# nilspin/VoxelHashing_demo

Measured on AMD Instinct MI355X. Metric: frames/s TSDF-integrated + raycast Mpix/s, 640×480, 1/2/4/8 MI355X, higher is better.
Workload: dtype f32

## Files before the change

voxelhashing_demo_amd/csrc/vh_api.hip:

```cpp
#include <hip/hip_runtime.h>
#include <hip/hip_ext.h>
#include <dlfcn.h>

#include <algorithm>
#include <chrono>
#include <cmath>
#include <cstdio>
#include <cstdlib>
#include <cstring>
#include <string>
#include <type_traits>
#include <utility>
#include <vector>

#include "vh_kernels.hip"

using namespace vh;

static thread_local std::string g_last_error;

static int fail(int code, const char *what, hipError_t e = hipSuccess)
{
    g_last_error = what;
    if (e != hipSuccess) {
// ... 143 lines not shown
    std::vector<std::pair<hipEvent_t, hipEvent_t>> eventPool;
    uint64_t profiledFrames = 0;
    vh_kernel_times times{};
    int integrateGrid = 2048;
    void *raycastStamps = nullptr;
    int raycastBeam = 3;
    int raycastMode = VH_RAYCAST_DDA;
    int packetFormat = VH_PACKET_F32;
    int fusedFrame = 1;
    int commitBlocks = 128;
    int fusedParity = 0;
    bool compactArmed = false;
    int flattenVariant = 4;
    int walkReverse = 1;
    uint32_t walkBackward = 0;
    uint32_t candAllocated = 0;
    uint32_t allocEpoch = 0;
    uint32_t epochTotal = 0;
    DevBuf<float> fusedPlane;
    int pipeline = 0;
    int pipeIntegrateGrid = 512;
    PendingFrame pend;
    int pipeSet = 0;
    int pipeParity = 0;
    unsigned long long *claimBuf[2] = {nullptr, nullptr};
    int4 *candBuf[2] = {nullptr, nullptr};
    VoxelEntry *compactBuf[2] = {nullptr, nullptr};
    DevBuf<uint32_t> claimFilter;
    DevBuf<uint32_t> maskBuf2;
    int genFramesPerLaunch = 4;
// ... 388 lines not shown
```

voxelhashing_demo_amd/csrc/vh_api_frame.hip:

```cpp

extern "C" int vh_reset_mutexes(vh_context *c)
{
    if (!c) return fail(VH_ERR_INVALID_ARGUMENT, "null context");
    if (c->fp.epoch >= kMaxClaimEpoch) {
        DeviceGuard guard(c->device);
        const int rc = flush_pending(c);
        if (rc != VH_OK) return rc;
        const size_t bytes = sizeof(unsigned long long) * (size_t)c->ownedBuckets;
        if (c->claimBuf[0]) {
            VH_HIP(hipMemsetAsync(c->claimBuf[0], 0, bytes, c->stream));
            VH_HIP(hipMemsetAsync(c->claimBuf[1], 0, bytes, c->stream));
        } else {
            VH_HIP(hipMemsetAsync(c->dp.claim, 0, bytes, c->stream));
        }
        c->fp.epoch = 0;
    }
    c->fp.epoch += 1;
    c->epochTotal += 1;
    return VH_OK;
}

static inline int grid_for(size_t n, int per_block) { return (int)((n + per_block - 1) / per_block); }
static inline uint32_t host_num_tiles(const vh_context *c)
{
// ... 49 lines not shown
{
    if (c->flattenVariant == kWalkIndexed)
        return (uint32_t)grid_for(((size_t)c->ownedBuckets + 31) / 32, kFlattenThreads * kIndexWords);
    return (uint32_t)grid_for(c->numEntries, kFlattenThreads * ((c->fp.flags & kFlagWalkShort) ? kEntriesPerLaneShort : kEntriesPerLane));
}

static inline uint32_t groups_of_8(uint32_t n) { return (n + 7u) / 8u; }
static uint32_t take_walk_direction(vh_context *c)
{
    const uint32_t reverse = c->walkReverse ? c->walkBackward : 0u;
    c->walkBackward ^= 1u;
    return reverse;
}

static bool multi_walk_indexed(const vh_context *c) { return c->flattenVariant == kWalkIndexed && !(c->fp.flags & kFlagOverflow); }
static bool multi_walk_short(const vh_context *c) { return c->numEntries * sizeof(VoxelEntry) >= ((size_t)32 << 20); }
static uint32_t multi_walk_blocks(const vh_context *c)
{
    return multi_walk_indexed(c) ? (uint32_t)grid_for(((size_t)c->ownedBuckets + 31) / 32, kFlattenThreads * kIndexWords)
                                 : (uint32_t)grid_for(c->numEntries, kFlattenThreads * (multi_walk_short(c) ? kEntriesPerLaneShort : kEntriesPerLane));
}

static uint32_t bin_parts(int32_t capacity) { return (uint32_t)std::max(1, grid_for((size_t)capacity, 256 * 4)); }

template <class F>
static int with_bool(bool b, F f) { return b ? f(std::true_type{}) : f(std::false_type{}); }

static int launch_flatten(vh_context *c)
{
    if (c->flattenVariant == kWalkIndexed)
        return launch(c, kPhaseFlatten, flatten_kernel<kWalkIndexed>, dim3(walk_blocks(c)), dim3(kFlattenThreads), c->fp, c->dp,
// ... 58 lines not shown
    VH_HIP(hipGetLastError());
    return VH_OK;
}

static uint32_t claim_span(const vh_context *c, uint32_t claimBlocks, uint32_t walkBlocks)
{
    const uint32_t total = claimBlocks + walkBlocks;
    const double walk_us = (double)c->numEntries * sizeof(VoxelEntry) / 6.0e6;
    double chain_us = 4.0;
    if (c->fp.allocBand > 0.0f)
        chain_us += 2.0 * std::min(8.0, 2.0 * std::ceil((double)c->fp.allocBand / (4.0 * c->fp.voxelSize)));
    const double share = std::min(1.0, std::max(0.5, 1.0 - chain_us / std::max(walk_us, 1.0)));
    return std::min(total, std::max<uint32_t>(claimBlocks + (walkBlocks ? 1u : 0u), (uint32_t)(share * total)));
}

static uint32_t claim_lead(const vh_context *c, uint32_t claimGroups, uint32_t walkGroups, uint32_t &span, bool pipelined)
{
    uint32_t want = 0u;
    if (c->claimLead >= 0) want = (uint32_t)c->claimLead;
    else if (pipelined && !(c->fp.allocBand > 0.0f)) {
        const size_t tileBytes = sizeof(VoxelEntry) * kFlattenThreads * ((c->fp.flags & kFlagWalkShort) ? kEntriesPerLaneShort : kEntriesPerLane);
        want = std::min<uint32_t>((uint32_t)(((size_t)4 << 20) / tileBytes), walkGroups / 4u);
    }
    const uint32_t least = claimGroups + (walkGroups ? 1u : 0u);
    const uint32_t lead = span > least ? std::min(want, span - least) : 0u;
    span -= lead;
    return lead;
}

static uint32_t claim_ratio(uint32_t claimBlocks, uint32_t span)
{
    if (span == 0 || claimBlocks >= span) return 0xffffffffu;
    return (uint32_t)((((uint64_t)claimBlocks << 32) + span - 1) / span);
}

static int ensure_pipeline_buffers(vh_context *c)
// ... 155 lines not shown
    a.commitBlocks = hasOld ? (uint32_t)c->commitBlocks : 0u;
    a.integrateBlocks = hasOld ? (uint32_t)c->pipeIntegrateGrid : 0u;
    if (hasOld && a.walkIndexed && large) a.integrateBlocks *= 2u;
    a.numEntries = (uint32_t)c->numEntries;
    a.walkGroups = 0u; a.walkReverse = 0u; a.claimLead = 0u;
    uint32_t claimWalk = a.claimBlocks + a.walkBlocks;
    if (a.walkIndexed) {
        a.claimSpan = claim_span(c, a.claimBlocks, a.walkBlocks);
        a.claimRatio = claim_ratio(a.claimBlocks, a.claimSpan);
    } else {
        a.commitBlocks = 8u * groups_of_8(a.commitBlocks);
        a.integrateBlocks = 8u * groups_of_8(a.integrateBlocks);
        const uint32_t claimGroups = groups_of_8(a.claimBlocks);
        a.walkGroups = groups_of_8(a.walkBlocks);
        a.claimSpan = claim_span(c, claimGroups, a.walkGroups);
        a.claimLead = claim_lead(c, claimGroups, a.walkGroups, a.claimSpan, true);
        a.claimRatio = claim_ratio(claimGroups, a.claimSpan);
        if (hasNew) a.walkReverse = take_walk_direction(c);
        claimWalk = 8u * (claimGroups + a.walkGroups);
    }
    args.planeNew = (hasNew && !newSensor) ? c->planeBuf[r.newParity].get() : nullptr;
    args.rawNew = (hasNew && newSensor) ? c->rawBuf[r.newParity].get() : nullptr;
    args.filter = c->claimFilter;
    args.filtNew = kPendFilterWords * (uint32_t)r.iNew; args.filtOld = kPendFilterWords * (uint32_t)r.iOld;
    args.filtClear = kPendFilterWords * (uint32_t)r.iClear;
#ifdef VH_DEBUG_SKIP_ROLES
    a.skipRoles = (uint32_t)c->debugSkipRoles;
#endif
    const dim3 grid(a.commitBlocks + a.integrateBlocks + claimWalk);
    In inNew{};
    if (hasNew) inNew = *in;
// ... 53 lines not shown

extern "C" int vh_flush(vh_context *c)
{
    VH_TRACE("vh_flush");
    if (!c) return fail(VH_ERR_INVALID_ARGUMENT, "null context");
    DeviceGuard guard(c->device);
    return settle(c);
}

template <int kKind, class In>
static int launch_scan_claim(vh_context *c, const In &in, uint32_t claimBlocks, uint32_t scanBlocks, float *planeOut)
{
    if (kKind != kWalkIndexed) {
        const uint32_t claimGroups = groups_of_8(claimBlocks), walkGroups = groups_of_8(scanBlocks);
        uint32_t span = claim_span(c, claimGroups, walkGroups);
        const uint32_t lead = claim_lead(c, claimGroups, walkGroups, span, false);
        return launch(c, kPhaseFrameScanClaim, frame_scan_claim_kernel<kKind, In>, dim3(8u * (claimGroups + walkGroups)),
                      dim3(256), c->fp, c->dp, in, (uint32_t)c->numEntries, claimBlocks, c->fusedParity, planeOut,
                      span, claim_ratio(claimGroups, span), walkGroups, take_walk_direction(c), lead);
    }
    return launch(c, kPhaseFrameScanClaim, frame_scan_claim_kernel<kKind, In>, dim3(claimBlocks + scanBlocks),
                  dim3(256), c->fp, c->dp, in, (uint32_t)c->numEntries, claimBlocks, c->fusedParity, planeOut,
                  claim_span(c, claimBlocks, scanBlocks), claim_ratio(claimBlocks, claim_span(c, claimBlocks, scanBlocks)), 0u, 0u, 0u);
}

static inline float *fused_plane(vh_context *c, const VertexMap &)
{
    if (!c->fusedPlane) (void)c->fusedPlane.try_alloc((size_t)c->fp.width * c->fp.height);
    return c->fusedPlane;
}
static inline float *fused_plane(vh_context *, const SensorImage &) { return nullptr; }
// ... 233 lines not shown
```

voxelhashing_demo_amd/csrc/vh_api_model.hip:

```cpp

static int sweep_and_release(vh_context *c)
{
    int rc;
    if (c->fp.flags & kFlagOverflow) {
        rc = launch(c, kPhaseGc, gc_sweep_overflow_a_kernel, dim3(256), dim3(256), c->fp, c->dp);
        if (rc == VH_OK) rc = launch(c, kPhaseGc, gc_sweep_overflow_b_kernel, dim3(256), dim3(256), c->fp, c->dp);
    } else {
        rc = launch(c, kPhaseGc, gc_sweep_kernel, dim3(256), dim3(256), c->fp, c->dp);
    }
    if (rc != VH_OK) return rc;
    rc = release_color(c);
    if (rc != VH_OK) return rc;
    rc = launch(c, kPhaseGc, gc_release_kernel, dim3(1024), dim3(256), c->dp);
    if (rc != VH_OK) return rc;
    rc = launch(c, kPhaseGc, gc_finish_kernel, dim3(1), dim3(1), c->dp, c->occupiedCounter);
    if (rc != VH_OK) return rc;
    if (c->profiling) c->times.gc_calls += 1;
    c->params.numOccupiedBlocks = 0;
    VH_HIP(hipGetLastError());
    return VH_OK;
}

extern "C" int vh_delete_blocks(vh_context *c, const int32_t *d_keys, int32_t n)
{
// ... 347 lines not shown
    if (c) { DeviceGuard fguard(c->device); const int frc = flush_pending(c); if (frc != VH_OK) return frc; }
    if (!c || !name) return fail(VH_ERR_INVALID_ARGUMENT, "null argument");
    if (std::strcmp(name, "flatten_variant") == 0) {
        if (value != kWalkStridedBallot && value != kWalkIndexed)
            return fail(VH_ERR_INVALID_ARGUMENT, "flatten_variant: 3 (the reference's walk) or 4 (occupancy index)");
        c->flattenVariant = value;
        return VH_OK;
    }
    if (std::strcmp(name, "walk_nt") == 0) {
        c->fp.flags = value ? (c->fp.flags | kFlagWalkNt) : (c->fp.flags & ~kFlagWalkNt);
        return VH_OK;
    }
    if (std::strcmp(name, "walk_reverse") == 0) { c->walkReverse = value != 0; return VH_OK; }
    if (std::strcmp(name, "walk_short") == 0) {
        c->fp.flags = value ? (c->fp.flags | kFlagWalkShort) : (c->fp.flags & ~kFlagWalkShort);
        return VH_OK;
    }
    if (std::strcmp(name, "claim_lead") == 0 && value >= -1) { c->claimLead = value; return VH_OK; }
#ifdef VH_DEBUG_SKIP_ROLES
    if (std::strcmp(name, "debug_skip_roles") == 0 && value >= 0 && value < 32) {
        c->debugSkipRoles = value;
        if (value & 16) c->fp.flags |= kFlagDebugNoProbe; else c->fp.flags &= ~kFlagDebugNoProbe;
        return VH_OK;
    }
#endif
    if (std::strcmp(name, "spin_limit") == 0 && value >= 0) { c->spinLimit = (uint32_t)value; return VH_OK; }
    if (std::strcmp(name, "pipeline_overflow") == 0 && value >= 0 && value <= 2) {
        DeviceGuard g(c->device);
        const int frc = flush_pending(c);
        if (frc != VH_OK) return frc;
// ... 147 lines not shown
```

voxelhashing_demo_amd/csrc/vh_api_shard.hip:

```cpp

static void make_view_frustum(const vh_context *c, const float pose[16], float t_min, float t_max, float f[22])
{
    float inv[16];
    invert4x4(pose, inv);
    std::memcpy(f, inv, 12 * sizeof(float));
    const float r = 7.0f * c->fp.voxelSize;
    const float a[4] = {(0.0f - c->rc_cx) / c->rc_fx, ((float)(c->fp.width - 1) - c->rc_cx) / c->rc_fx,
                        (0.0f - c->rc_cy) / c->rc_fy, ((float)(c->fp.height - 1) - c->rc_cy) / c->rc_fy};
    for (int i = 0; i < 4; ++i) {
        f[12 + i] = a[i];
        f[16 + i] = -(r * sqrtf(1.0f + a[i] * a[i]));
    }
    f[20] = t_min - r;
    f[21] = t_max + r;
}

extern "C" int vh_export_views(vh_context *c, const float *poses, int32_t n_views, float t_min, float t_max,
                               vh_view_record *d_records, int32_t capacity, int32_t *d_counts)
{
    if (!c || !poses || !d_records || !d_counts) return fail(VH_ERR_INVALID_ARGUMENT, "null argument");
    if (n_views < 1 || n_views > VH_MAX_CAMERAS) return fail(VH_ERR_INVALID_ARGUMENT, "1..VH_MAX_CAMERAS views");
    if (capacity < 1) return fail(VH_ERR_INVALID_ARGUMENT, "capacity must be positive");
    if (!(t_max > t_min)) return fail(VH_ERR_INVALID_ARGUMENT, "t_max must exceed t_min");
    if (c->viewBlocks) return fail(VH_ERR_INVALID_ARGUMENT, "a view table has no voxels of its own to export");
// ... 302 lines not shown
        for (int j = 0; j < n; ++j) {
            const int rc = vh_set_pose(c, poses + 16 * (size_t)(b0 + j));
            if (rc != VH_OK) return rc;
            if (!d_depth[b0 + j]) return fail(VH_ERR_INVALID_ARGUMENT, "null depth image");
            std::memcpy(fr.T[j], c->fp.T, sizeof fr.T[j]);
            std::memcpy(fr.Tinv[j], c->fp.Tinv, sizeof fr.Tinv[j]);
            fr.depth[j] = d_depth[b0 + j];
        }
        write_packets_u16_kernel<<<dim3(64, (unsigned)n), 256, 0, c->stream>>>(
            fr, (int32_t)npix, d_packets + packet_frame_stride * (size_t)b0, packet_frame_stride);
    }
    VH_HIP(hipGetLastError());
    return VH_OK;
}

struct MultiBatch {
    const int4 *bins;
    const float *packets;
    int32_t numBins, capacity, binStride, frameStride, numCams;
    size_t packetStride, packetFrameStride;
    bool perBatch;
};

static int launch_multi_pipelined(vh_context *c, const MultiBatch *mb, int b, const GenJob *job)
{
    PendingFrame &pend = c->pend;
    const bool doNew = mb != nullptr, hasOld = pend.kind == PendingFrame::kMulti;
    if (!doNew && !hasOld) return VH_OK;
    int rc;
    if (doNew && (rc = vh_reset_mutexes(c)) != VH_OK) return rc;
    uint32_t *maskOf[2] = {c->dp.compactMask, c->maskBuf2};
    MultiPipeArgs a;
    std::memset(&a, 0, sizeof a);
    PipeRotation r = pipe_rotation(c, a, a, doNew, hasOld);
    a.numEntries = (uint32_t)c->numEntries;
    a.numCams = doNew ? mb->numCams : pend.numCams;
    a.packetStride = doNew ? mb->packetStride : pend.packetStride;
    if (doNew) {
        a.partsPerBin = bin_parts(mb->capacity); a.numBins = (uint32_t)mb->numBins;
        a.claimBlocks = a.numBins * a.partsPerBin;
        a.walkShort = multi_walk_short(c) ? 1u : 0u;
        a.walkIndexed = multi_walk_indexed(c) ? 1u : 0u;
        a.walkBlocks = multi_walk_blocks(c);
        a.capacity = mb->capacity; a.binStride = mb->binStride;
        a.binsNew = mb->bins + (size_t)mb->frameStride * b;
        a.binFrame = mb->perBatch ? b : -1;
        a.packetsNew = mb->packets + mb->packetFrameStride * b;
    }
    a.commitBlocks = hasOld ? (uint32_t)c->commitBlocks : 0u;
    a.integrateBlocks = hasOld ? (uint32_t)c->pipeIntegrateGrid : 0u;
    a.claimSpan = claim_span(c, a.claimBlocks, a.walkBlocks);
    a.claimRatio = claim_ratio(a.claimBlocks, a.claimSpan);
    a.epochOld = pend.epoch;
    a.packetsOld = pend.packets;
    r.dpNew.compactMask = maskOf[r.newParity];
    a.claimOld = r.dpOld.claim; a.candOld = r.dpOld.candidates; a.compactOld = r.dpOld.compact; a.maskOld = maskOf[r.oldParity];
    a.candCapacityOld = r.dpOld.candCapacity;
    const bool sensor = (doNew ? c->packetFormat : pend.packetFormat) == VH_PACKET_U16;
    const bool serial = (c->fp.flags & kFlagOverflow) != 0u;
    const bool gen = job && job->blocks && doNew && sensor && !serial;
    if (gen) a.gen = *job;
    const dim3 grid(a.commitBlocks + a.integrateBlocks + (gen ? a.gen.blocks : 0u) + a.claimBlocks + a.walkBlocks);
    using Yes = std::true_type;
    using No = std::false_type;
    auto go = [&](auto sensorC, auto serialC, auto indexedC, auto genC) {
        return launch(c, kPhaseFramePipelined,
                      frame_multi_pipelined_kernel<decltype(sensorC)::value, decltype(serialC)::value, decltype(indexedC)::value, decltype(genC)::value>,
                      grid, dim3(256), c->fp, r.dpNew, a);
    };
    if (gen) rc = with_bool(a.walkIndexed != 0u, [&](auto i) { return go(Yes{}, No{}, i, Yes{}); });
    else if (a.walkIndexed) rc = with_bool(sensor, [&](auto s) { return go(s, No{}, Yes{}, No{}); });
    else rc = with_bool(sensor, [&](auto s) { return with_bool(serial, [&](auto q) { return go(s, q, No{}, No{}); }); });
    if (rc != VH_OK) return rc;
    pipe_launched(c, r, serial, doNew ? PendingFrame::kMulti : PendingFrame::kNone, hasOld, false, hasOld);
    if (doNew) {
        pend.epoch = c->fp.epoch;
        pend.packets = a.packetsNew;
        pend.packetStride = mb->packetStride;
        pend.numCams = mb->numCams;
        pend.packetFormat = c->packetFormat;
    }
    return VH_OK;
}

static bool multi_can_pipeline(const vh_context *c, int32_t num_bins, int32_t capacity)
{
    return can_pipeline(c, (uint32_t)num_bins * bin_parts(capacity) + (uint32_t)grid_for(c->numEntries, kFlattenThreads * kEntriesPerLaneShort));
}

static bool multi_can_fuse_generation(const vh_context *c, int32_t num_bins, int32_t capacity)
{
    return c->pipelineShards && multi_can_pipeline(c, num_bins, capacity) && !(c->fp.flags & kFlagOverflow) &&
           c->packetFormat == VH_PACKET_U16 && !(c->fp.allocBand > 0.0f) && c->flattenVariant != kWalkIndexed;
}

static bool multi_fusing_pays(const vh_context *c)
{
    return (size_t)c->numEntries * sizeof(VoxelEntry) > ((size_t)60 << 20);
}

static int vh_apply_frames_batch_gen(vh_context *c, int32_t batch, const int32_t *d_bins, int32_t num_bins,
                                     int32_t capacity, int32_t bin_stride, int32_t frame_stride, int32_t num_cams,
// ... 142 lines not shown
```

voxelhashing_demo_amd/csrc/vh_frame.hip:

```cpp
#pragma once

namespace vh {

__device__ __forceinline__ bool grouped_role(uint32_t r, uint32_t claimBlocks, uint32_t claimSpan, uint32_t claimRatio,
                                             uint32_t claimLead, uint32_t &index)
{
    const uint32_t g = (r >> 3) - claimLead, q = r & 7u;
    uint32_t before = (int32_t)g < 0 ? 0u : (claimBlocks + 7u) >> 3;
    if (g < claimSpan) {
        const unsigned long long phase = (unsigned long long)q << 29;
        before = (uint32_t)(((unsigned long long)g * claimRatio + phase) >> 32);
        const uint32_t after = (uint32_t)(((unsigned long long)(g + 1u) * claimRatio + phase) >> 32);
        if (after != before) { index = 8u * before + q; return true; }
    }
    index = r - 8u * before;
    return false;
}

template <int kKind, class In>
__global__ __launch_bounds__(256) void frame_scan_claim_kernel(const FrameParams fp, const DevPtrs dp, const In in,
                                                               uint32_t numEntries, uint32_t claimBlocks,
                                                               int parity, float *__restrict__ planeOut, uint32_t claimSpan,
                                                               uint32_t claimRatio, uint32_t walkGroups, uint32_t walkReverse,
                                                               uint32_t claimLead)
// ... 164 lines not shown
struct PipeKernargs {
    FrameParams fpNew;
    DevPtrs dpNew;
    In inNew;
    FrameParams fpOld;
    DevPtrs dpOld;
    Depth depthOld;
    PipeArgs a;
};
template <class In, class Depth>
struct PipeSignature {
    PipeLeadWords lead;
    PipeKernargs<In, Depth> rest;
};

template <class In, class Depth, int kLean>
__device__ __forceinline__ const PipeKernargs<In, Depth> &role_arguments()
{
    typedef PipeKernargs<In, Depth> K;
    typedef PipeSignature<In, Depth> Signature;
    static_assert(offsetof(Signature, lead) == 0 && offsetof(Signature, rest) == sizeof(PipeLeadWords),
                  "frame_pipelined_kernel(lead, rest): rest lies right behind lead");
    typedef const __attribute__((address_space(4))) char *SegmentBytes;
    typedef const __attribute__((address_space(4))) K *SegmentPtr;
    SegmentPtr p = (SegmentPtr)((SegmentBytes)__builtin_amdgcn_kernarg_segment_ptr() + offsetof(Signature, rest));
    asm volatile("" : "+s"(p));
    const K &k = *(const K *)p;
    constexpr uint32_t leanFlags = lean_build(kLean).flags;
    if (kLean != kLeanNone) {
        __builtin_assume(k.fpNew.flags == leanFlags);
        __builtin_assume(k.fpOld.flags == leanFlags);
    }
    return k;
}

template <class In, class Depth, bool kBand, bool kSerial, int kLean>
__device__ __forceinline__ void frame_pipelined(const PipeLead &l)
{
    typedef PipeKernargs<In, Depth> K;
    constexpr LeanBuild lean = lean_build(kLean);
    const bool walkIndexed = kLean != kLeanNone ? lean.indexed : l.walkIndexed != 0u;
    constexpr bool serial = kSerial;
// ... 168 lines not shown
```

voxelhashing_demo_amd/csrc/vh_shard.hip:

```cpp
#pragma once

namespace vh {

constexpr int kBinFrameMarks = 0x40000000;

__device__ __forceinline__ void claim_bin_slice(const FrameParams &fp, const DevPtrs &dp,
                                                const int4 *__restrict__ bins, int32_t capacity, int32_t binStride,
                                                uint32_t binIndex, uint32_t part, uint32_t parts, int candCounter,
                                                const Pending &pend = kNoPending, int frame = -1)
{
    const int4 *bin = bins + (size_t)binIndex * binStride;
    const int4 head = bin[0];
    int n = head.x;
    const bool frameMarks = frame >= 0 && (head.w & kBinFrameMarks) != 0;
    const int room = frameMarks ? capacity - 3 : capacity - 1;
    int lo = 0, hiMark = 0;
    if (frameMarks) {
        const int4 c0 = bin[capacity - 2], c1 = bin[capacity - 1];
        const int cnt[8] = {c0.x, c0.y, c0.z, c0.w, c1.x, c1.y, c1.z, c1.w};
        n = 0;
#pragma unroll
        for (int f = 0; f < 8; ++f) {
            if (f == frame) lo = n;
            n += cnt[f];
            if (f == frame) hiMark = n;
        }
    }
// ... 14 lines not shown
#ifdef VH_DEBUG_SKIP_ROLES
    if (fp.flags & kFlagDebugNoProbe) n = min(n, lo + ((n - lo) >> 5));
#endif
    for (int i = lo + (int)part * 256 + (int)threadIdx.x; i < n; i += (int)parts * 256) {
        const int4 k = bin[1 + i];
        uint32_t rank = (uint32_t)k.w;
        if (frame >= 0) {
            if ((rank >> kRankCameraShift) != (uint32_t)frame) continue;
            rank = (binIndex << kRankCameraShift) | (rank & ((1u << kRankCameraShift) - 1u));
        }
        const uint32_t h = hash_block(k.x, k.y, k.z, fp.numBuckets);
        if (h < fp.bucketLo || h >= fp.bucketHi) continue;
        probe_and_claim(fp, dp, k.x, k.y, k.z, h, rank, candCounter, pend);
    }
}

__global__ __launch_bounds__(256) void claim_bins_kernel(const FrameParams fp, const DevPtrs dp,
                                                         const int4 *__restrict__ bins, int32_t capacity,
                                                         int32_t binStride)
{
    claim_bin_slice(fp, dp, bins, capacity, binStride, blockIdx.y, blockIdx.x, gridDim.x, kCandCount);
}

__device__ __forceinline__ uint32_t camera_mask(const FrameParams &fp, const int *pos, int32_t numCams,
                                                const float *__restrict__ packets, size_t packetStride)
{
    uint32_t seen = 0;
    for (int c = 0; c < numCams; ++c) {
        const float *pk = packets + packetStride * c;
        if (block_in_frustum(fp, pk, pk + 16, pos[0], pos[1], pos[2])) seen |= 1u << c;
    }
    return seen;
}

template <int kN = kEntriesPerLane>
__device__ __forceinline__ void flatten_multi_tile(const FrameParams &fp, const DevPtrs &dp, uint32_t numEntries,
                                                   uint32_t tileIndex, int32_t numCams,
                                                   const float *__restrict__ packets, size_t packetStride,
                                                   int counter, const Pending &pend = kNoPending)
{
    const uint32_t tile = tileIndex * (kFlattenThreads * kN);
    int32_t ptrs[kN];
    walk_load_tile(fp, dp, numEntries, tileIndex, ptrs);
    uint32_t seen[kN];
    int myCount = 0;
#pragma unroll
    for (int j = 0; j < kN; ++j) {
        seen[j] = 0;
        if (ptrs[j] == VH_FREE_BLOCK) continue;
        const uint32_t e = tile + j * kFlattenThreads + threadIdx.x;
        const VoxelEntry ent = dp.table[e];
        if (pend.claim && pend.live) {
            const uint32_t b = e / fp.bucketSize;
            const unsigned long long w = pend.claim[b];
            if (claim_epoch(w) == pend.epoch && claim_f(w) == e - b * fp.bucketSize) continue;
        }
        seen[j] = camera_mask(fp, ent.pos, numCams, packets, packetStride);
        myCount += seen[j] != 0u;
    }
    int slot = reserve_compact_slots(dp, counter, myCount);
    if (slot < 0) return;
#pragma unroll
    for (int j = 0; j < kN; ++j) {
        if (seen[j] == 0u) continue;
        dp.compact[slot] = dp.table[tile + j * kFlattenThreads + threadIdx.x];
        dp.compactMask[slot] = seen[j];
        ++slot;
    }
}

struct IndexSinkMulti {
    const FrameParams &fp;
    int32_t numCams;
    const float *__restrict__ packets;
    size_t packetStride;
    int counterIndex;
    __device__ __forceinline__ uint32_t judge(const VoxelEntry &e) const { return camera_mask(fp, e.pos, numCams, packets, packetStride); }
    __device__ __forceinline__ int counter() const { return counterIndex; }
    __device__ __forceinline__ void emit(const DevPtrs &dp, uint32_t pos, const VoxelEntry &e, uint32_t seen) const
    {
        dp.compact[pos] = e;
        dp.compactMask[pos] = seen;
    }
// ... 115 lines not shown
constexpr int kFusedGenGroups = VH_FUSED_GEN_GROUPS;
struct GenJob {
    uint32_t blocks;
    int32_t numShards, capacity, binStride;
    int4 *bins;
    float *packet;
    const uint16_t *depth;
    uint32_t rankBase;
    float T[16], Tinv[16], k[9], unit;
    int4 *clearBins;
    int32_t clearStride;
    int32_t frame, batch;
};


struct MultiPipeArgs {
    uint32_t claimBlocks, walkBlocks, commitBlocks, integrateBlocks;
    uint32_t partsPerBin, numBins, numEntries;
    int32_t capacity, binStride, numCams;
    int32_t binFrame;
    int32_t doneTag;
    uint32_t spinLimit;
    int32_t setNew, setOld, setClear;
    uint32_t hasNew, hasOld;
    uint32_t walkShort;
    uint32_t walkIndexed;
    uint32_t claimSpan, claimRatio;
    uint32_t epochOld;
    const int4 *binsNew;
    const float *packetsNew, *packetsOld;
    size_t packetStride;
    unsigned long long *claimOld;
    int4 *candOld;
    VoxelEntry *compactOld;
    uint32_t *maskOld;
    uint32_t candCapacityOld;
    GenJob gen;
};

template <bool kSensor, bool kSerial, bool kIndexed = false, bool kGen = false>
__global__ __launch_bounds__(256) void frame_multi_pipelined_kernel(const FrameParams fp, const DevPtrs dp, const MultiPipeArgs a)
{
    if (!a.hasOld && blockIdx.x == 0u && threadIdx.x == 0) dp.counters[kPipeHeapFree + a.setNew] = dp.counters[kHeapCounter] + 1;
    if constexpr (kGen) {
        const uint32_t g0 = a.commitBlocks + a.integrateBlocks;
        if (blockIdx.x >= g0 && blockIdx.x < g0 + a.gen.blocks) {
            const uint32_t g = blockIdx.x - g0;
            if (VH_FUSED_GEN_PRIO) __builtin_amdgcn_s_setprio(VH_FUSED_GEN_PRIO);
            FrameParams fg = fp;
#pragma unroll
            for (int i = 0; i < 16; ++i) { fg.T[i] = a.gen.T[i]; fg.Tinv[i] = a.gen.Tinv[i]; }
            SensorImage in;
            in.depth = a.gen.depth;
#pragma unroll
            for (int i = 0; i < 9; ++i) in.k[i] = a.gen.k[i];
            in.unit = a.gen.unit;
            float *pk = a.gen.packet;
            if (g == 0 && threadIdx.x < kPacketHeaderU16) {
                const int t = threadIdx.x;
                pk[t] = t < 16 ? a.gen.T[t] : t < 32 ? a.gen.Tinv[t - 16] : t == 32 ? a.gen.k[6] : t == 33 ? a.gen.k[7] : t == 34 ? a.gen.k[8] : a.gen.unit;
            }
            if (g == 0 && a.gen.clearBins && (int)threadIdx.x < a.gen.numShards) {
                int4 *nb = a.gen.clearBins + (size_t)threadIdx.x * a.gen.clearStride;
                nb[0] = make_int4(0, 0, 0, kBinFrameMarks | a.gen.batch);
                nb[a.gen.capacity - 2] = make_int4(0, 0, 0, 0);
                nb[a.gen.capacity - 1] = make_int4(0, 0, 0, 0);
            }
#pragma unroll
            for (int j = 0; j < kFusedGenGroups; ++j) {
                const int idx = ((int)g * kFusedGenGroups + j) * 256 + (int)threadIdx.x;
                if (idx < fp.width * fp.height) reinterpret_cast<uint16_t *>(pk + kPacketHeaderU16)[idx] = in.depth[idx];
            }
            generate_keys_groups<SensorImage, 256, kFusedGenGroups>(fg, in, a.gen.numShards, a.gen.bins, a.gen.capacity - 2, a.gen.binStride, nullptr,
                                                                    a.gen.rankBase, g * (uint32_t)kFusedGenGroups, a.gen.frame);
            return;
        }
    }
    const uint32_t genBlocks = kGen ? a.gen.blocks : 0u;
    int32_t *counters = dp.counters;
    const int demandedOld = a.hasOld ? counters[kPipeCand + a.setOld] : 0;
    const int candOld = min(demandedOld, (int)a.candCapacityOld);
    constexpr bool serial = kSerial;
    const bool live = serial ? a.hasOld != 0u : a.hasOld && counters[kPipeHeapFree + a.setOld] >= counters[kPipeWinners + a.setOld];
    const uint32_t b = blockIdx.x;
    if (b >= a.commitBlocks + a.integrateBlocks + genBlocks) {
        if (!a.hasNew) return;
        if (serial && a.hasOld) {
            if (!wait_commit_done(counters, a.doneTag, a.spinLimit)) return;
        }
        const Pending pend{a.hasOld && !serial ? a.claimOld : nullptr, a.candOld, a.epochOld, live, serial ? -1 : kPipeWinners + a.setNew};
        const uint32_t r = b - a.commitBlocks - a.integrateBlocks - genBlocks;
        uint32_t before = a.claimBlocks, after = a.claimBlocks;
        if constexpr (kIndexed) {
            if (r < a.walkBlocks) {
                flatten_index_tile_to(fp, dp, r, IndexSinkMulti{fp, a.numCams, a.packetsNew, a.packetStride, kPipeScan + a.setNew}, pend);
                return;
            }
            before = r - a.walkBlocks; after = before + 1u;
        }
        else { if (r < a.claimSpan) { before = __umulhi(r, a.claimRatio); after = __umulhi(r + 1u, a.claimRatio); } }
        if (after != before) {
            __builtin_amdgcn_s_setprio(3);
            claim_bin_slice(fp, dp, a.binsNew, a.capacity, a.binStride, before / a.partsPerBin, before % a.partsPerBin, a.partsPerBin,
                            kPipeCand + a.setNew, pend, a.binFrame);
        } else {
            if (a.walkShort) flatten_multi_tile<kEntriesPerLaneShort>(fp, dp, a.numEntries, r - before, a.numCams, a.packetsNew, a.packetStride, kPipeScan + a.setNew, pend);
            else flatten_multi_tile(fp, dp, a.numEntries, r - before, a.numCams, a.packetsNew, a.packetStride, kPipeScan + a.setNew, pend);
        }
        return;
    }
    if (!a.hasOld) return;
    const int scanOld = counters[kPipeScan + a.setOld];
    if (b >= a.commitBlocks) {
        for (int k = (int)(b - a.commitBlocks); k < scanOld; k += (int)a.integrateBlocks)
            integrate_block_multi<kSensor>(fp, dp, a.compactOld[k], a.maskOld[k], a.numCams, a.packetsOld, a.packetStride);
        return;
    }
    __shared__ VoxelEntry newEntry;
    __shared__ uint32_t newMask;
    __shared__ int inserted;
    const int workers = max(1, min(candOld, (int)a.commitBlocks));
    if ((int)b >= workers) return;
    for (int i = (int)b; i < candOld; i += (int)a.commitBlocks) {
        if (threadIdx.x == 0) {
            inserted = 0;
            newMask = 0u;
            const int4 k = a.candOld[i];
            if (live) {
                VoxelEntry e;
                inserted = commit_candidate(fp, dp, k, e, (uint32_t)i, false, a.epochOld, a.claimOld) ? 1 : 0;
                if (inserted) {
                    const uint32_t seen = camera_mask(fp, e.pos, a.numCams, a.packetsOld, a.packetStride);
                    newEntry = e;
                    newMask = seen;
                    if (seen != 0u) {
                        const int slot = scanOld + atomicAdd(counters + kPipeNew + a.setOld, 1);
                        a.compactOld[slot] = e;
                        a.maskOld[slot] = seen;
                    }
                    if (a.hasNew && !serial) {
                        const uint32_t next = camera_mask(fp, e.pos, a.numCams, a.packetsNew, a.packetStride);
                        if (next != 0u) {
                            const int slot = atomicAdd(counters + kPipeScan + a.setNew, 1);
                            dp.compact[slot] = e;
                            dp.compactMask[slot] = next;
                        }
                    }
                }
            } else {
                const uint32_t local = hash_block(k.x, k.y, k.z, fp.numBuckets) - fp.bucketLo;
                const unsigned long long w = a.claimOld[local];
                if (claim_epoch(w) == a.epochOld && claim_slot(w) == (uint32_t)i) atomicAdd(counters + kHeapExhausted, 1);
            }
        }
        __syncthreads();
        if (inserted && newMask != 0u)
            integrate_block_multi<kSensor>(fp, dp, newEntry, newMask, a.numCams, a.packetsOld, a.packetStride);
        __syncthreads();
    }
    if (threadIdx.x == 0) {
        __threadfence();
        const int ticket = atomicAdd(counters + kCommitTicket, 1);
        if (ticket == workers - 1) {
            counters[kCompactCount] = scanOld + atomicAdd(counters + kPipeNew + a.setOld, 0);
            counters[kLastCandidates] = demandedOld;
            clear_pipe_set(counters, a.setClear);
            if (!a.hasNew) clear_pipe_set(counters, a.setNew);
            counters[kPipeHeapFree + a.setNew] = atomicAdd(counters + kHeapCounter, 0) + 1;
            counters[kCommitTicket] = 0;
            if (serial) {
                __threadfence();
                __hip_atomic_store(counters + kPipeCommitDone, a.doneTag, __ATOMIC_RELAXED, __HIP_MEMORY_SCOPE_AGENT);
            }
        }
    }
}

struct SensorFrames {
    float T[kGenBatch][16];
    float Tinv[kGenBatch][16];
    const uint16_t *depth[kGenBatch];
    float k6, k7, k8, unit;
};

__global__ __launch_bounds__(256) void write_packets_u16_kernel(const SensorFrames fr, int32_t numPixels,
                                                                float *__restrict__ packets, size_t packetFrameStride)
{
    const int b = blockIdx.y;
    float *pk = packets + packetFrameStride * b;
    if (blockIdx.x == 0 && threadIdx.x < kPacketHeaderU16) {
        const int t = threadIdx.x;
// ... 38 lines not shown
```

Measured before the change: 64870.

## Port lead-word kernargs and grouped claim/walk roles to multi-camera pipelined kernel

Reworks the multi-camera pipelined frame kernel to take a 64-byte lead struct of role-dispatch scalars ahead of the bulk arguments. Each block can then pick its role and start its walk table loads before it reads the rest of the kernarg segment. The claim/walk dispatch moves from a per-block ratio split to grouped-of-8 roles with walk direction alternation, claim lead, and rounded commit/integrate/gen block counts, matching the single-camera path. Walk tile size now follows an explicit override knob. The risk is extra complexity from reading kernargs through raw segment pointers, and different block scheduling interplay between claims and walks.

Result: no change. 64910, median of 3 (+0.1%).

```diff
diff --git a/voxelhashing_demo_amd/csrc/vh_api.hip b/voxelhashing_demo_amd/csrc/vh_api.hip
--- a/voxelhashing_demo_amd/csrc/vh_api.hip
+++ b/voxelhashing_demo_amd/csrc/vh_api.hip
@@ -181,6 +181,7 @@
     int flattenVariant = 4;
     int walkReverse = 1;
     uint32_t walkBackward = 0;
+    int multiWalkShort = -1;
     uint32_t candAllocated = 0;
     uint32_t allocEpoch = 0;
     uint32_t epochTotal = 0;
diff --git a/voxelhashing_demo_amd/csrc/vh_api_frame.hip b/voxelhashing_demo_amd/csrc/vh_api_frame.hip
--- a/voxelhashing_demo_amd/csrc/vh_api_frame.hip
+++ b/voxelhashing_demo_amd/csrc/vh_api_frame.hip
@@ -87,7 +87,11 @@
 }
 
 static bool multi_walk_indexed(const vh_context *c) { return c->flattenVariant == kWalkIndexed && !(c->fp.flags & kFlagOverflow); }
-static bool multi_walk_short(const vh_context *c) { return c->numEntries * sizeof(VoxelEntry) >= ((size_t)32 << 20); }
+static bool multi_walk_short(const vh_context *c)
+{
+    if (c->multiWalkShort >= 0) return c->multiWalkShort != 0;
+    return c->numEntries * sizeof(VoxelEntry) >= ((size_t)32 << 20);
+}
 static uint32_t multi_walk_blocks(const vh_context *c)
 {
     return multi_walk_indexed(c) ? (uint32_t)grid_for(((size_t)c->ownedBuckets + 31) / 32, kFlattenThreads * kIndexWords)
@@ -176,12 +180,12 @@
     return std::min(total, std::max<uint32_t>(claimBlocks + (walkBlocks ? 1u : 0u), (uint32_t)(share * total)));
 }
 
-static uint32_t claim_lead(const vh_context *c, uint32_t claimGroups, uint32_t walkGroups, uint32_t &span, bool pipelined)
+static uint32_t claim_lead(const vh_context *c, uint32_t claimGroups, uint32_t walkGroups, uint32_t &span, bool pipelined, bool shortTiles)
 {
     uint32_t want = 0u;
     if (c->claimLead >= 0) want = (uint32_t)c->claimLead;
     else if (pipelined && !(c->fp.allocBand > 0.0f)) {
-        const size_t tileBytes = sizeof(VoxelEntry) * kFlattenThreads * ((c->fp.flags & kFlagWalkShort) ? kEntriesPerLaneShort : kEntriesPerLane);
+        const size_t tileBytes = sizeof(VoxelEntry) * kFlattenThreads * (shortTiles ? kEntriesPerLaneShort : kEntriesPerLane);
         want = std::min<uint32_t>((uint32_t)(((size_t)4 << 20) / tileBytes), walkGroups / 4u);
     }
     const uint32_t least = claimGroups + (walkGroups ? 1u : 0u);
@@ -367,7 +371,7 @@
         const uint32_t claimGroups = groups_of_8(a.claimBlocks);
         a.walkGroups = groups_of_8(a.walkBlocks);
         a.claimSpan = claim_span(c, claimGroups, a.walkGroups);
-        a.claimLead = claim_lead(c, claimGroups, a.walkGroups, a.claimSpan, true);
+        a.claimLead = claim_lead(c, claimGroups, a.walkGroups, a.claimSpan, true, (c->fp.flags & kFlagWalkShort) != 0u);
         a.claimRatio = claim_ratio(claimGroups, a.claimSpan);
         if (hasNew) a.walkReverse = take_walk_direction(c);
         claimWalk = 8u * (claimGroups + a.walkGroups);
@@ -451,7 +455,7 @@
     if (kKind != kWalkIndexed) {
         const uint32_t claimGroups = groups_of_8(claimBlocks), walkGroups = groups_of_8(scanBlocks);
         uint32_t span = claim_span(c, claimGroups, walkGroups);
-        const uint32_t lead = claim_lead(c, claimGroups, walkGroups, span, false);
+        const uint32_t lead = claim_lead(c, claimGroups, walkGroups, span, false, (c->fp.flags & kFlagWalkShort) != 0u);
         return launch(c, kPhaseFrameScanClaim, frame_scan_claim_kernel<kKind, In>, dim3(8u * (claimGroups + walkGroups)),
                       dim3(256), c->fp, c->dp, in, (uint32_t)c->numEntries, claimBlocks, c->fusedParity, planeOut,
                       span, claim_ratio(claimGroups, span), walkGroups, take_walk_direction(c), lead);
diff --git a/voxelhashing_demo_amd/csrc/vh_api_model.hip b/voxelhashing_demo_amd/csrc/vh_api_model.hip
--- a/voxelhashing_demo_amd/csrc/vh_api_model.hip
+++ b/voxelhashing_demo_amd/csrc/vh_api_model.hip
@@ -385,6 +385,7 @@
     if (std::strcmp(name, "walk_reverse") == 0) { c->walkReverse = value != 0; return VH_OK; }
     if (std::strcmp(name, "walk_short") == 0) {
         c->fp.flags = value ? (c->fp.flags | kFlagWalkShort) : (c->fp.flags & ~kFlagWalkShort);
+        c->multiWalkShort = value ? 1 : 0;
         return VH_OK;
     }
     if (std::strcmp(name, "claim_lead") == 0 && value >= -1) { c->claimLead = value; return VH_OK; }
diff --git a/voxelhashing_demo_amd/csrc/vh_api_shard.hip b/voxelhashing_demo_amd/csrc/vh_api_shard.hip
--- a/voxelhashing_demo_amd/csrc/vh_api_shard.hip
+++ b/voxelhashing_demo_amd/csrc/vh_api_shard.hip
@@ -340,6 +340,8 @@
     return VH_OK;
 }
 
+constexpr bool kMultiClaimLeadRule = false;
+
 struct MultiBatch {
     const int4 *bins;
     const float *packets;
@@ -358,25 +360,26 @@
     uint32_t *maskOf[2] = {c->dp.compactMask, c->maskBuf2};
     MultiPipeArgs a;
     std::memset(&a, 0, sizeof a);
-    PipeRotation r = pipe_rotation(c, a, a, doNew, hasOld);
-    a.numEntries = (uint32_t)c->numEntries;
+    MultiPipeLead l{};
+    PipeRotation r = pipe_rotation(c, a, l, doNew, hasOld);
+    l.table = r.dpNew.table;
+    l.numEntries = (uint32_t)c->numEntries;
     a.numCams = doNew ? mb->numCams : pend.numCams;
     a.packetStride = doNew ? mb->packetStride : pend.packetStride;
+    const bool indexed = doNew && multi_walk_indexed(c);
+    const bool shortTiles = multi_walk_short(c);
     if (doNew) {
         a.partsPerBin = bin_parts(mb->capacity); a.numBins = (uint32_t)mb->numBins;
-        a.claimBlocks = a.numBins * a.partsPerBin;
-        a.walkShort = multi_walk_short(c) ? 1u : 0u;
-        a.walkIndexed = multi_walk_indexed(c) ? 1u : 0u;
-        a.walkBlocks = multi_walk_blocks(c);
+        l.claimBlocks = a.numBins * a.partsPerBin;
+        l.walkFlags = (shortTiles ? kFlagWalkShort : 0u) | (c->fp.flags & kFlagWalkNt);
+        l.walkBlocks = multi_walk_blocks(c);
         a.capacity = mb->capacity; a.binStride = mb->binStride;
         a.binsNew = mb->bins + (size_t)mb->frameStride * b;
         a.binFrame = mb->perBatch ? b : -1;
         a.packetsNew = mb->packets + mb->packetFrameStride * b;
     }
-    a.commitBlocks = hasOld ? (uint32_t)c->commitBlocks : 0u;
-    a.integrateBlocks = hasOld ? (uint32_t)c->pipeIntegrateGrid : 0u;
-    a.claimSpan = claim_span(c, a.claimBlocks, a.walkBlocks);
-    a.claimRatio = claim_ratio(a.claimBlocks, a.claimSpan);
+    l.commitBlocks = hasOld ? (uint32_t)c->commitBlocks : 0u;
+    l.integrateBlocks = hasOld ? (uint32_t)c->pipeIntegrateGrid : 0u;
     a.epochOld = pend.epoch;
     a.packetsOld = pend.packets;
     r.dpNew.compactMask = maskOf[r.newParity];
@@ -385,17 +388,34 @@
     const bool sensor = (doNew ? c->packetFormat : pend.packetFormat) == VH_PACKET_U16;
     const bool serial = (c->fp.flags & kFlagOverflow) != 0u;
     const bool gen = job && job->blocks && doNew && sensor && !serial;
-    if (gen) a.gen = *job;
-    const dim3 grid(a.commitBlocks + a.integrateBlocks + (gen ? a.gen.blocks : 0u) + a.claimBlocks + a.walkBlocks);
+    if (gen) { a.gen = *job; l.genBlocks = job->blocks; }
+    uint32_t genBlocks = l.genBlocks, claimWalk = l.claimBlocks + l.walkBlocks;
+    if (indexed) {
+        l.claimSpan = claim_span(c, l.claimBlocks, l.walkBlocks);
+        l.claimRatio = claim_ratio(l.claimBlocks, l.claimSpan);
+    } else {
+        l.commitBlocks = 8u * groups_of_8(l.commitBlocks);
+        l.integrateBlocks = 8u * groups_of_8(l.integrateBlocks);
+        genBlocks = 8u * groups_of_8(genBlocks);
+        const uint32_t claimGroups = groups_of_8(l.claimBlocks);
+        l.walkGroups = groups_of_8(l.walkBlocks);
+        l.claimSpan = claim_span(c, claimGroups, l.walkGroups);
+        l.claimLead = claim_lead(c, claimGroups, l.walkGroups, l.claimSpan, kMultiClaimLeadRule, shortTiles);
+        l.claimRatio = claim_ratio(claimGroups, l.claimSpan);
+        if (doNew) l.walkReverse = take_walk_direction(c);
+        claimWalk = 8u * (claimGroups + l.walkGroups);
+    }
+    const dim3 grid(l.commitBlocks + l.integrateBlocks + genBlocks + claimWalk);
+    const MultiPipeSignature sig{__builtin_bit_cast(PipeLeadWords, l), {c->fp, r.dpNew, a}};
     using Yes = std::true_type;
     using No = std::false_type;
     auto go = [&](auto sensorC, auto serialC, auto indexedC, auto genC) {
         return launch(c, kPhaseFramePipelined,
                       frame_multi_pipelined_kernel<decltype(sensorC)::value, decltype(serialC)::value, decltype(indexedC)::value, decltype(genC)::value>,
-                      grid, dim3(256), c->fp, r.dpNew, a);
+                      grid, dim3(256), sig.lead, sig.rest);
     };
-    if (gen) rc = with_bool(a.walkIndexed != 0u, [&](auto i) { return go(Yes{}, No{}, i, Yes{}); });
-    else if (a.walkIndexed) rc = with_bool(sensor, [&](auto s) { return go(s, No{}, Yes{}, No{}); });
+    if (gen) rc = with_bool(indexed, [&](auto i) { return go(Yes{}, No{}, i, Yes{}); });
+    else if (indexed) rc = with_bool(sensor, [&](auto s) { return go(s, No{}, Yes{}, No{}); });
     else rc = with_bool(sensor, [&](auto s) { return with_bool(serial, [&](auto q) { return go(s, q, No{}, No{}); }); });
     if (rc != VH_OK) return rc;
     pipe_launched(c, r, serial, doNew ? PendingFrame::kMulti : PendingFrame::kNone, hasOld, false, hasOld);
@@ -411,7 +431,8 @@
 
 static bool multi_can_pipeline(const vh_context *c, int32_t num_bins, int32_t capacity)
 {
-    return can_pipeline(c, (uint32_t)num_bins * bin_parts(capacity) + (uint32_t)grid_for(c->numEntries, kFlattenThreads * kEntriesPerLaneShort));
+    const uint32_t claims = (uint32_t)num_bins * bin_parts(capacity), walks = multi_walk_blocks(c);
+    return can_pipeline(c, multi_walk_indexed(c) ? claims + walks : 8u * (groups_of_8(claims) + groups_of_8(walks)));
 }
 
 static bool multi_can_fuse_generation(const vh_context *c, int32_t num_bins, int32_t capacity)
diff --git a/voxelhashing_demo_amd/csrc/vh_frame.hip b/voxelhashing_demo_amd/csrc/vh_frame.hip
--- a/voxelhashing_demo_amd/csrc/vh_frame.hip
+++ b/voxelhashing_demo_amd/csrc/vh_frame.hip
@@ -202,18 +202,23 @@
     PipeKernargs<In, Depth> rest;
 };
 
-template <class In, class Depth, int kLean>
-__device__ __forceinline__ const PipeKernargs<In, Depth> &role_arguments()
-{
-    typedef PipeKernargs<In, Depth> K;
-    typedef PipeSignature<In, Depth> Signature;
+template <class Signature>
+__device__ __forceinline__ auto arguments_behind_lead() -> const decltype(Signature::rest) &
+{
+    typedef decltype(Signature::rest) K;
     static_assert(offsetof(Signature, lead) == 0 && offsetof(Signature, rest) == sizeof(PipeLeadWords),
-                  "frame_pipelined_kernel(lead, rest): rest lies right behind lead");
+                  "kernel(lead, rest): rest lies right behind lead");
     typedef const __attribute__((address_space(4))) char *SegmentBytes;
     typedef const __attribute__((address_space(4))) K *SegmentPtr;
     SegmentPtr p = (SegmentPtr)((SegmentBytes)__builtin_amdgcn_kernarg_segment_ptr() + offsetof(Signature, rest));
     asm volatile("" : "+s"(p));
-    const K &k = *(const K *)p;
+    return *(const K *)p;
+}
+template <class In, class Depth, int kLean>
+__device__ __forceinline__ const PipeKernargs<In, Depth> &role_arguments()
+{
+    typedef PipeKernargs<In, Depth> K;
+    const K &k = arguments_behind_lead<PipeSignature<In, Depth>>();
     constexpr uint32_t leanFlags = lean_build(kLean).flags;
     if (kLean != kLeanNone) {
         __builtin_assume(k.fpNew.flags == leanFlags);
diff --git a/voxelhashing_demo_amd/csrc/vh_shard.hip b/voxelhashing_demo_amd/csrc/vh_shard.hip
--- a/voxelhashing_demo_amd/csrc/vh_shard.hip
+++ b/voxelhashing_demo_amd/csrc/vh_shard.hip
@@ -4,13 +4,10 @@
 
 constexpr int kBinFrameMarks = 0x40000000;
 
-__device__ __forceinline__ void claim_bin_slice(const FrameParams &fp, const DevPtrs &dp,
-                                                const int4 *__restrict__ bins, int32_t capacity, int32_t binStride,
-                                                uint32_t binIndex, uint32_t part, uint32_t parts, int candCounter,
-                                                const Pending &pend = kNoPending, int frame = -1)
-{
-    const int4 *bin = bins + (size_t)binIndex * binStride;
-    const int4 head = bin[0];
+__device__ __forceinline__ void claim_bin_records(const FrameParams &fp, const DevPtrs &dp, const int4 *bin,
+                                                  const int4 head, int32_t capacity, uint32_t binIndex, uint32_t part,
+                                                  uint32_t parts, int candCounter, const Pending &pend, int frame)
+{
     int n = head.x;
     const bool frameMarks = frame >= 0 && (head.w & kBinFrameMarks) != 0;
     const int room = frameMarks ? capacity - 3 : capacity - 1;
@@ -55,6 +52,14 @@
         probe_and_claim(fp, dp, k.x, k.y, k.z, h, rank, candCounter, pend);
     }
 }
+__device__ __forceinline__ void claim_bin_slice(const FrameParams &fp, const DevPtrs &dp,
+                                                const int4 *__restrict__ bins, int32_t capacity, int32_t binStride,
+                                                uint32_t binIndex, uint32_t part, uint32_t parts, int candCounter,
+                                                const Pending &pend = kNoPending, int frame = -1)
+{
+    const int4 *bin = bins + (size_t)binIndex * binStride;
+    claim_bin_records(fp, dp, bin, bin[0], capacity, binIndex, part, parts, candCounter, pend, frame);
+}
 
 __global__ __launch_bounds__(256) void claim_bins_kernel(const FrameParams fp, const DevPtrs dp,
                                                          const int4 *__restrict__ bins, int32_t capacity,
@@ -74,15 +79,13 @@
     return seen;
 }
 
-template <int kN = kEntriesPerLane>
-__device__ __forceinline__ void flatten_multi_tile(const FrameParams &fp, const DevPtrs &dp, uint32_t numEntries,
-                                                   uint32_t tileIndex, int32_t numCams,
+template <int kN>
+__device__ __forceinline__ void flatten_multi_list(const FrameParams &fp, const DevPtrs &dp, uint32_t tileIndex,
+                                                   const int32_t (&ptrs)[kN], int32_t numCams,
                                                    const float *__restrict__ packets, size_t packetStride,
-                                                   int counter, const Pending &pend = kNoPending)
+                                                   int counter, const Pending &pend)
 {
     const uint32_t tile = tileIndex * (kFlattenThreads * kN);
-    int32_t ptrs[kN];
-    walk_load_tile(fp, dp, numEntries, tileIndex, ptrs);
     uint32_t seen[kN];
     int myCount = 0;
 #pragma unroll
@@ -108,6 +111,16 @@
         dp.compactMask[slot] = seen[j];
         ++slot;
     }
+}
+template <int kN = kEntriesPerLane>
+__device__ __forceinline__ void flatten_multi_tile(const FrameParams &fp, const DevPtrs &dp, uint32_t numEntries,
+                                                   uint32_t tileIndex, int32_t numCams,
+                                                   const float *__restrict__ packets, size_t packetStride,
+                                                   int counter, const Pending &pend = kNoPending)
+{
+    int32_t ptrs[kN];
+    walk_load_tile(fp, dp, numEntries, tileIndex, ptrs);
+    flatten_multi_list(fp, dp, tileIndex, ptrs, numCams, packets, packetStride, counter, pend);
 }
 
 struct IndexSinkMulti {
@@ -253,18 +266,26 @@
 };
 
 
+struct MultiPipeLead {
+    uint32_t commitBlocks, integrateBlocks, claimBlocks, walkBlocks;
+    uint32_t genBlocks;
+    uint32_t claimSpan, claimRatio;
+    uint32_t claimLead;
+    uint32_t walkGroups, walkReverse;
+    uint32_t walkFlags;
+    uint32_t numEntries;
+    uint32_t hasNew, hasOld;
+    const VoxelEntry *table;
+};
+static_assert(sizeof(MultiPipeLead) == sizeof(PipeLeadWords), "MultiPipeLead is the one 64-byte scalar load at the head of the arguments");
+
 struct MultiPipeArgs {
-    uint32_t claimBlocks, walkBlocks, commitBlocks, integrateBlocks;
-    uint32_t partsPerBin, numBins, numEntries;
+    uint32_t partsPerBin, numBins;
     int32_t capacity, binStride, numCams;
     int32_t binFrame;
     int32_t doneTag;
     uint32_t spinLimit;
     int32_t setNew, setOld, setClear;
-    uint32_t hasNew, hasOld;
-    uint32_t walkShort;
-    uint32_t walkIndexed;
-    uint32_t claimSpan, claimRatio;
     uint32_t epochOld;
     const int4 *binsNew;
     const float *packetsNew, *packetsOld;
@@ -277,14 +298,32 @@
     GenJob gen;
 };
 
-template <bool kSensor, bool kSerial, bool kIndexed = false, bool kGen = false>
-__global__ __launch_bounds__(256) void frame_multi_pipelined_kernel(const FrameParams fp, const DevPtrs dp, const MultiPipeArgs a)
-{
-    if (!a.hasOld && blockIdx.x == 0u && threadIdx.x == 0) dp.counters[kPipeHeapFree + a.setNew] = dp.counters[kHeapCounter] + 1;
+struct MultiPipeKernargs {
+    FrameParams fp;
+    DevPtrs dp;
+    MultiPipeArgs a;
+};
+struct MultiPipeSignature {
+    PipeLeadWords lead;
+    MultiPipeKernargs rest;
+};
+
+template <bool kSensor, bool kSerial, bool kIndexed, bool kGen>
+__device__ __forceinline__ void frame_multi_pipelined(const MultiPipeLead &l)
+{
+    typedef MultiPipeKernargs K;
+    const auto arguments = []() -> const K & { return arguments_behind_lead<MultiPipeSignature>(); };
+    const uint32_t deferred = l.commitBlocks + l.integrateBlocks;
+    constexpr bool serial = kSerial;
+    const uint32_t b = blockIdx.x;
+    const uint32_t genBlocks = !kGen ? 0u : kIndexed ? l.genBlocks : (l.genBlocks + 7u) & ~7u;
     if constexpr (kGen) {
-        const uint32_t g0 = a.commitBlocks + a.integrateBlocks;
-        if (blockIdx.x >= g0 && blockIdx.x < g0 + a.gen.blocks) {
-            const uint32_t g = blockIdx.x - g0;
+        if (b >= deferred && b < deferred + genBlocks) {
+            const uint32_t g = b - deferred;
+            if (g >= l.genBlocks) return;
+            const K &k = arguments();
+            const FrameParams &fp = k.fp;
+            const MultiPipeArgs &a = k.a;
             if (VH_FUSED_GEN_PRIO) __builtin_amdgcn_s_setprio(VH_FUSED_GEN_PRIO);
             FrameParams fg = fp;
 #pragma unroll
@@ -315,52 +354,84 @@
             return;
         }
     }
-    const uint32_t genBlocks = kGen ? a.gen.blocks : 0u;
+    if (b >= deferred + genBlocks) {
+        if (!l.hasNew) return;
+        const uint32_t r = b - deferred - genBlocks;
+        uint32_t index;
+        bool claims;
+        if constexpr (kIndexed) {
+            claims = r >= l.walkBlocks;
+            index = claims ? r - l.walkBlocks : r;
+        } else {
+            claims = grouped_role(r, l.claimBlocks, l.claimSpan, l.claimRatio, l.claimLead, index);
+            if (claims ? index >= l.claimBlocks : walk_tile(index, l.walkGroups, l.walkReverse) >= l.walkBlocks) return;
+        }
+        if (serial && l.hasOld) {
+            const K &k = arguments();
+            if (!wait_commit_done(k.dp.counters, k.a.doneTag, k.a.spinLimit)) return;
+        }
+        const auto pending = [&](const K &k) {
+            return Pending{l.hasOld && !serial ? k.a.claimOld : nullptr, k.a.candOld, k.a.epochOld,
+                           pending_live<serial>(l.hasOld, k.dp.counters, k.a.setOld), serial ? -1 : kPipeWinners + k.a.setNew};
+        };
+        if (!claims && !kIndexed) {
+            const uint32_t tile = walk_tile(index, l.walkGroups, l.walkReverse);
+            typedef const __attribute__((address_space(1))) VoxelEntry *GlobalTable;
+            FrameParams loadFp{};
+            DevPtrs loadDp{};
+            loadFp.flags = l.walkFlags;
+            loadDp.table = (VoxelEntry *)(GlobalTable)(uintptr_t)l.table;
+            const auto walk = [&](auto &ptrs) {
+                walk_load_tile(loadFp, loadDp, l.numEntries, tile, ptrs);
+                if (!walk_wave_live(ptrs)) return;
+                const K &k = arguments();
+                flatten_multi_list(k.fp, k.dp, tile, ptrs, k.a.numCams, k.a.packetsNew, k.a.packetStride, kPipeScan + k.a.setNew, pending(k));
+            };
+            if (l.walkFlags & kFlagWalkShort) {
+                int32_t ptrs[kEntriesPerLaneShort];
+                walk(ptrs);
+            } else {
+                int32_t ptrs[kEntriesPerLane];
+                walk(ptrs);
+            }
+            return;
+        }
+        const K &k = arguments();
+        const MultiPipeArgs &a = k.a;
+        if (!claims) {
+            flatten_index_tile_to(k.fp, k.dp, index, IndexSinkMulti{k.fp, a.numCams, a.packetsNew, a.packetStride, kPipeScan + a.setNew}, pending(k));
+            return;
+        }
+        __builtin_amdgcn_s_setprio(3);
+        const uint32_t binIndex = index / a.partsPerBin, part = index % a.partsPerBin;
+        const int4 *bin = a.binsNew + (size_t)binIndex * a.binStride;
+        const int4 head = bin[0];
+        if (!l.hasOld && index == 0u && threadIdx.x == 0) k.dp.counters[kPipeHeapFree + a.setNew] = k.dp.counters[kHeapCounter] + 1;
+        claim_bin_records(k.fp, k.dp, bin, head, a.capacity, binIndex, part, a.partsPerBin, kPipeCand + a.setNew, pending(k), a.binFrame);
+        return;
+    }
+    if (!l.hasOld) return;
+    const K &k = arguments();
+    const FrameParams &fp = k.fp;
+    const DevPtrs &dp = k.dp;
+    const MultiPipeArgs &a = k.a;
     int32_t *counters = dp.counters;
-    const int demandedOld = a.hasOld ? counters[kPipeCand + a.setOld] : 0;
+    if (b >= l.commitBlocks) {
+        const int scanOld = counters[kPipeScan + a.setOld];
+        for (int i = (int)(b - l.commitBlocks); i < scanOld; i += (int)l.integrateBlocks)
+            integrate_block_multi<kSensor>(fp, dp, a.compactOld[i], a.maskOld[i], a.numCams, a.packetsOld, a.packetStride);
+        return;
+    }
+    const int demandedOld = counters[kPipeCand + a.setOld];
+    const int scanOld = counters[kPipeScan + a.setOld];
+    const bool live = pending_live<serial>(l.hasOld, counters, a.setOld);
     const int candOld = min(demandedOld, (int)a.candCapacityOld);
-    constexpr bool serial = kSerial;
-    const bool live = serial ? a.hasOld != 0u : a.hasOld && counters[kPipeHeapFree + a.setOld] >= counters[kPipeWinners + a.setOld];
-    const uint32_t b = blockIdx.x;
-    if (b >= a.commitBlocks + a.integrateBlocks + genBlocks) {
-        if (!a.hasNew) return;
-        if (serial && a.hasOld) {
-            if (!wait_commit_done(counters, a.doneTag, a.spinLimit)) return;
-        }
-        const Pending pend{a.hasOld && !serial ? a.claimOld : nullptr, a.candOld, a.epochOld, live, serial ? -1 : kPipeWinners + a.setNew};
-        const uint32_t r = b - a.commitBlocks - a.integrateBlocks - genBlocks;
-        uint32_t before = a.claimBlocks, after = a.claimBlocks;
-        if constexpr (kIndexed) {
-            if (r < a.walkBlocks) {
-                flatten_index_tile_to(fp, dp, r, IndexSinkMulti{fp, a.numCams, a.packetsNew, a.packetStride, kPipeScan + a.setNew}, pend);
-                return;
-            }
-            before = r - a.walkBlocks; after = before + 1u;
-        }
-        else { if (r < a.claimSpan) { before = __umulhi(r, a.claimRatio); after = __umulhi(r + 1u, a.claimRatio); } }
-        if (after != before) {
-            __builtin_amdgcn_s_setprio(3);
-            claim_bin_slice(fp, dp, a.binsNew, a.capacity, a.binStride, before / a.partsPerBin, before % a.partsPerBin, a.partsPerBin,
-                            kPipeCand + a.setNew, pend, a.binFrame);
-        } else {
-            if (a.walkShort) flatten_multi_tile<kEntriesPerLaneShort>(fp, dp, a.numEntries, r - before, a.numCams, a.packetsNew, a.packetStride, kPipeScan + a.setNew, pend);
-            else flatten_multi_tile(fp, dp, a.numEntries, r - before, a.numCams, a.packetsNew, a.packetStride, kPipeScan + a.setNew, pend);
-        }
-        return;
-    }
-    if (!a.hasOld) return;
-    const int scanOld = counters[kPipeScan + a.setOld];
-    if (b >= a.commitBlocks) {
-        for (int k = (int)(b - a.commitBlocks); k < scanOld; k += (int)a.integrateBlocks)
-            integrate_block_multi<kSensor>(fp, dp, a.compactOld[k], a.maskOld[k], a.numCams, a.packetsOld, a.packetStride);
-        return;
-    }
     __shared__ VoxelEntry newEntry;
     __shared__ uint32_t newMask;
     __shared__ int inserted;
-    const int workers = max(1, min(candOld, (int)a.commitBlocks));
+    const int workers = max(1, min(candOld, (int)l.commitBlocks));
     if ((int)b >= workers) return;
-    for (int i = (int)b; i < candOld; i += (int)a.commitBlocks) {
+    for (int i = (int)b; i < candOld; i += (int)l.commitBlocks) {
         if (threadIdx.x == 0) {
             inserted = 0;
             newMask = 0u;
@@ -377,7 +448,7 @@
                         a.compactOld[slot] = e;
                         a.maskOld[slot] = seen;
                     }
-                    if (a.hasNew && !serial) {
+                    if (l.hasNew && !serial) {
                         const uint32_t next = camera_mask(fp, e.pos, a.numCams, a.packetsNew, a.packetStride);
                         if (next != 0u) {
                             const int slot = atomicAdd(counters + kPipeScan + a.setNew, 1);
@@ -404,7 +475,7 @@
             counters[kCompactCount] = scanOld + atomicAdd(counters + kPipeNew + a.setOld, 0);
             counters[kLastCandidates] = demandedOld;
             clear_pipe_set(counters, a.setClear);
-            if (!a.hasNew) clear_pipe_set(counters, a.setNew);
+            if (!l.hasNew) clear_pipe_set(counters, a.setNew);
             counters[kPipeHeapFree + a.setNew] = atomicAdd(counters + kHeapCounter, 0) + 1;
             counters[kCommitTicket] = 0;
             if (serial) {
@@ -414,6 +485,18 @@
         }
     }
 }
+
+#pragma clang diagnostic push
+#pragma clang diagnostic ignored "-Wpsabi"
+template <bool kSensor, bool kSerial, bool kIndexed = false, bool kGen = false>
+__global__ __launch_bounds__(256) void frame_multi_pipelined_kernel(const PipeLeadWords lead, const MultiPipeKernargs)
+{
+    static_assert(std::is_same<decltype(MultiPipeSignature::lead), PipeLeadWords>::value &&
+                  std::is_same<decltype(MultiPipeSignature::rest), MultiPipeKernargs>::value, "keep MultiPipeSignature in step");
+    const MultiPipeLead l = __builtin_bit_cast(MultiPipeLead, lead);
+    frame_multi_pipelined<kSensor, kSerial, kIndexed, kGen>(l);
+}
+#pragma clang diagnostic pop
 
 struct SensorFrames {
     float T[kGenBatch][16];
```
